# fulcrumgenomics/fgumi

Hardware: AMD Instinct MI355X
Metric: simplex consensus throughput, input raw reads/s (depth-8 x 150bp) (higher is better)
Workload: dtype f64

## Files before the change

### fgumi_amd/csrc/fastpath.hip

```cpp
#if !defined(FGX_WAVEMU)
#include <hipcub/hipcub.hpp>
#endif
#include "bamrec.h"
#include "canon_core.h"
#include "engine.h"
#include <cstdlib>
#include <memory>
#include <string>
#include <type_traits>
#include "fastpath.h"
#include "gate_core.h"
#include "packed_core.h"

#if defined(FGX_WAVEMU)
#define FGX_DYN_LDS(name) uint8_t* const name = wavemu::dyn_lds()
#define FGX_PIN(...) ((void)0)
#define FGX_UNDEF4(a, b, c, d) do { a = 0; b = 0; c = 0; d = 0; } while (0)
#define FGX_MEM_PIN() ((void)0)
#define FGX_CONST_AS
#else
#define FGX_DYN_LDS(name) extern __shared__ __align__(16) uint8_t name[]
#define FGX_PIN(...) asm volatile("" : __VA_ARGS__)
#define FGX_UNDEF4(a, b, c, d) asm volatile("" : "=v"(a), "=v"(b), "=v"(c), "=v"(d))
#define FGX_MEM_PIN() asm volatile("" ::: "memory")
// ... 3219 lines not shown
      FGX_LAUNCH(k_call_full, dim3((mx + 255) / 256, N_LISTS), dim3(256), 0, s, F);
    }
    if (meth_dev) FGX_LAUNCH(k_meth_sizes, dim3((n_slots + 3) / 4), dim3(256), 0, s, P, n_slots, fp.d_mslot.as<MethSlot>());
    if (meth_dup) FGX_LAUNCH(k_duplex_meth_sizes, dim3((n_slots + 3) / 4), dim3(256), 0, s, P, n_slots, fp.d_mslot.as<DuplexMethSlot>());
    return 0;
  }

  int check_direct() {
    FGX_LAUNCH(k_fix_ce, dim3((n_slots + 255) / 256), dim3(256), 0, s, fp.d_slot_desc.as<SlotDesc>(), fp.d_slot_err.as<uint32_t>(), n_slots, fp.d_out.as<uint8_t>(), P.rg_len);
    unsigned long long h_flags = 0, h_def = 0, h_route = 0;
    hip_check(hipMemcpyAsync(&h_flags, misc + MISC_DIR_FLAGS, 8, hipMemcpyDeviceToHost, s), "D2H");
    hip_check(hipMemcpyAsync(&h_def, misc + MISC_N_DEFERRED, 8, hipMemcpyDeviceToHost, s), "D2H");
    hip_check(hipMemcpyAsync(&h_route, misc + MISC_N_ROUTE, 8, hipMemcpyDeviceToHost, s), "D2H");
    hip_check(hipMemcpyAsync(&dir_total, fp.d_dir_base.as<uint64_t>() + fp.dir_chunks_run, 8, hipMemcpyDeviceToHost, s), "D2H");
    sync();
    if ((uint32_t)h_flags != 0) {
      fprintf(stderr, "[fgx] direct records: %u families differ in size from the prediction; this caller goes back to the column scratch (please report)\n", (uint32_t)h_flags);
      fp.direct_off = true;
      return FastPath::RUN_AGAIN_LARGER_POOL;
    }
    if ((uint32_t)(h_flags >> 32) != 0) {
      fp.dir_cap_min = dir_total + dir_total / 16 + 4096;
      if (ps.verbose) fprintf(stderr, "[fgx] direct records: the batch needs %llu bytes of output, %llu were at hand: again\n", (unsigned long long)dir_total, (unsigned long long)dir_cap);
      return FastPath::RUN_AGAIN_LARGER_POOL;
    }
    dir_routed = (uint32_t)h_route;
    dir_pure = dir_routed == 0 && (uint32_t)h_def == 0;
    fp.last_direct = dir_pure ? 1 : 2;
    if (ps.verbose) fprintf(stderr, "[fgx] direct records: %llu bytes in place, %u families left the split pipeline, %u deferred\n", (unsigned long long)dir_total, dir_routed, (uint32_t)h_def);
    return 0;
  }

  void place_records() {
    hip_check(hipEventRecord(fp.ev[1], s), "event");
    out_len = dir_total;
    out_ptr = fp.d_out.as<uint8_t>();
    if (dir_pure) return;
    scan_u64(fp.d_sizes.as<uint64_t>(), fp.d_offsets.as<uint64_t>(), n_slots + 1, "scan");
    uint64_t out_total = 0;
    hip_check(hipMemcpyAsync(&out_total, fp.d_offsets.as<uint64_t>() + n_slots, 8, hipMemcpyDeviceToHost, s), "D2H");
    sync();
    out_len = out_total;
    if (out_len > (1ull << 40)) throw std::runtime_error("device pipeline: the scan of the record sizes gives " + std::to_string(out_len) + " bytes of output (a record size is corrupt)");
    if (direct) { fp.d_out2.reserve(out_len + 16); out_ptr = fp.d_out2.as<uint8_t>(); }
    else { fp.d_out.reserve(out_len + 16); out_ptr = fp.d_out.as<uint8_t>(); }
  }

  template <class EP, class Desc> void emit_params(EP& E, const Desc* ends, uint8_t* out) const {
    memset(&E, 0, sizeof(E));
    E.blob = d_blob; E.rec_off = d_rec_off; E.ends = ends; E.out_off = fp.d_offsets.as<uint64_t>(); E.out = out;
    E.slot_end = n_slots;
    E.col_code = P.col_code; E.col_qual = P.col_qual; E.col_err = P.col_err;
    E.prefix = fp.d_strings.as<char>(); E.prefix_len = P.prefix_len; E.rg = fp.d_strings.as<char>() + P.prefix_len; E.rg_len = P.rg_len;
    E.per_base_tags = P.per_base_tags; E.cell0 = P.cell0; E.cell1 = P.cell1;
  }
  void write_records() {
    hip_check(hipEventRecord(fp.ev[2], s), "event");
    const dim3 per_slot((n_slots + 255) / 256), wave_per_slot((n_slots + 3) / 4), wave_per_family((n_grp + 3) / 4);
    DuplexEmitParams DE;
    CodecEmitParams CE;
    if (codec) {
      emit_params(CE, fp.d_ends.as<CodecDesc>(), fp.d_out.as<uint8_t>());
      CE.col_depth = P.col_depth;
      CE.has_outer = o.codec_has_outer_bases_qual; CE.outer_qual = o.codec_outer_bases_qual; CE.outer_len = o.codec_outer_bases_length;
      CE.has_ss = o.codec_has_single_strand_qual; CE.ss_qual = o.codec_single_strand_qual;
      CE.stats = fp.d_statslots.as<unsigned long long>();
      CE.n_slow = cnt(MISC_N_SLOW);
      FGX_LAUNCH(HIP_KERNEL_NAME(k_count_slow<CodecDesc>), per_slot, dim3(256), 0, s, CE.ends, 0u, n_slots, CE.prefix_len, CE.rg_len, CE.n_slow);
      FGX_LAUNCH(k_emit_codec_fast, wave_per_slot, dim3(256), 0, s, CE);
    } else if (duplex) {
      emit_params(DE, fp.d_ends.as<DuplexDesc>(), fp.d_out.as<uint8_t>());
      DE.col_obs = P.col_obs;
      DE.n_slow = cnt(MISC_N_SLOW);
      DE.meth_flag = P.meth_flag;
      DE.col_obs_all = P.col_obs_all;
      FGX_LAUNCH(HIP_KERNEL_NAME(k_count_slow<DuplexDesc>), per_slot, dim3(256), 0, s, DE.ends, 0u, n_slots, DE.prefix_len, DE.rg_len, DE.n_slow);
      if (meth_dup) FGX_LAUNCH(HIP_KERNEL_NAME(k_emit_duplex_fast<1>), wave_per_slot, dim3(256), 0, s, DE);
      else if (dup_cap) FGX_LAUNCH(HIP_KERNEL_NAME(k_emit_duplex_fast<0, 1>), wave_per_slot, dim3(256), 0, s, DE);
      else FGX_LAUNCH(HIP_KERNEL_NAME(k_emit_duplex_fast<0>), wave_per_slot, dim3(256), 0, s, DE);
    } else if (!direct || !dir_pure) {
      EmitParams E;
      emit_params(E, fp.d_ends.as<EndDesc>(), out_ptr);
      E.col_depth = P.col_depth; E.tag0 = P.tag0; E.tag1 = P.tag1;
      if (!direct) FGX_LAUNCH(k_emit, wave_per_family, dim3(256), 0, s, E);
      else {
        if (dir_routed) {
          E.fam_list = fp.d_route.as<uint32_t>(); E.n_fam = dir_routed;
          FGX_LAUNCH(k_emit, dim3((dir_routed + 3) / 4), dim3(256), 0, s, E);
        }
        FGX_LAUNCH(k_dir_copy, wave_per_family, dim3(256), 0, s, fp.d_split_out.as<SplitOut>(), fp.d_dir_off.as<uint64_t>(), fp.d_offsets.as<uint64_t>(),
                   fp.d_sizes.as<uint64_t>(), fp.d_out.as<uint8_t>(), out_ptr, n_grp);
      }
    }
    if (meth_dev) FGX_LAUNCH(k_meth_tail, wave_per_slot, dim3(256), 0, s, P, n_slots, fp.d_mslot.as<MethSlot>(), fp.d_offsets.as<uint64_t>(), out_ptr);
    if (meth_dup) FGX_LAUNCH(k_duplex_meth_tail, wave_per_slot, dim3(256), 0, s, P, n_slots, fp.d_mslot.as<DuplexMethSlot>(), fp.d_offsets.as<uint64_t>(), out_ptr);
    hip_check(hipEventRecord(fp.ev[3], s), "event");
    hip_check(hipEventRecord(c->ev1, s), "event");
    unsigned long long h_misc[MISC_READ_BACK];
    auto read_counters = [&] {
      FGX_LAUNCH(k_reduce_stats, dim3(1), dim3(64), 0, s, fp.d_statslots.as<unsigned long long>(), misc);
      hip_check(hipMemcpyAsync(h_misc, misc, sizeof(h_misc), hipMemcpyDeviceToHost, s), "D2H");
      sync();
    };
    read_counters();
    if ((duplex || codec) && (uint32_t)h_misc[MISC_N_SLOW] != 0) {
      if (codec) FGX_LAUNCH(k_emit_codec, wave_per_slot, dim3(256), 0, s, CE);
      else if (meth_dup) FGX_LAUNCH(HIP_KERNEL_NAME(k_emit_duplex<1>), wave_per_slot, dim3(256), 0, s, DE);
      else if (dup_cap) FGX_LAUNCH(HIP_KERNEL_NAME(k_emit_duplex<0, 1>), wave_per_slot, dim3(256), 0, s, DE);
      else FGX_LAUNCH(HIP_KERNEL_NAME(k_emit_duplex<0>), wave_per_slot, dim3(256), 0, s, DE);
      read_counters();
    }
    float ms = 0, msf = 0, mse = 0;
    hip_check(hipEventElapsedTime(&ms, c->ev0, c->ev1), "elapsed");
    hip_check(hipEventElapsedTime(&msf, fp.ev[0], fp.ev[1]), "elapsed");
    hip_check(hipEventElapsedTime(&mse, fp.ev[2], fp.ev[3]), "elapsed");
    res->d_out = out_ptr;
    res->out_len = out_len;
    res->count = h_misc[MISC_STATS + 1];
    for (int i = 0; i < FGX_STATS_LEN; i++) res->stats[i] = h_misc[MISC_STATS + i];
    res->n_deferred = (uint32_t)(h_misc[MISC_N_DEFERRED] & 0xFFFFFFFFull);
    fp.last_meth_clipped = (uint32_t)(h_misc[MISC_N_METH_CLIPPED] & 0xFFFFFFFFull);
    res->d_deferred = fp.d_deferred.as<uint32_t>();
    res->d_out_off = fp.d_offsets.as<uint64_t>();
    res->d_slot_size = fp.d_sizes.as<uint64_t>();
    res->n_slots = n_slots;
    res->ms_kernels = ms; res->ms_k_family = msf; res->ms_k_emit = mse;
    fp.last_packed_families = h_misc[MISC_BUILD_FAMILIES]; fp.last_classic_families = h_misc[MISC_BUILD_FAMILIES + 1];
    fp.last_packed_clean = h_misc[MISC_BUILD_FAMILIES + 2]; fp.last_packed_general = h_misc[MISC_BUILD_FAMILIES + 3];
    res->cols_used = h_misc[MISC_COLS_USED];
    res->full_items = n_full;
  }
};

int run_once(FastPath& fp, fgx_caller* c, const uint8_t* d_blob, uint64_t blob_len, const uint64_t* d_rec_off, const uint32_t* d_rec_len, uint32_t n_rec,
             const uint32_t* d_grp_first, uint32_t n_grp, FastResult* res) {
  memset(res, 0, sizeof(*res));
  fp.last_launches = 0; fp.last_host_syncs = 0;
  if (n_grp == 0) return 0;
  static const ProcessSwitches ps{};
  Batch b{fp, c, d_blob, blob_len, d_rec_off, d_rec_len, n_rec, d_grp_first, n_grp, res, ps};
  b.set_up();
  b.parse_first_chunk_early();
  b.bound_columns();
  b.fill_params();
  if (b.use_split) b.split_pipeline();
  if (b.simplex_v2) b.wave2_chain();
  b.family_wave_stages();
  b.deep_families();
  b.workgroup_families();
  if (const int rc = b.call_full()) return rc;
  if (b.direct) if (const int rc = b.check_direct()) return rc;
  b.place_records();
  b.write_records();
  return 0;
}

}

int FastPath::run(fgx_caller* c, const uint8_t* d_blob, uint64_t blob_len, const uint64_t* d_rec_off, const uint32_t* d_rec_len,
                  uint32_t n_rec, const uint32_t* d_grp_first, uint32_t n_grp, FastResult* res) {
  if (!pool_init) {
    if (const char* e = getenv("FGX_POOL_DIV")) { const long v = atol(e); if (v >= 1 && v <= (1 << 20)) pool_div = (uint32_t)v; }
    if (const char* e = getenv("FGX_POOL_SLACK")) { const long v = atol(e); if (v >= 1 && v <= 4096) pool_slack = (uint32_t)v; }
    pool_init = true;
  }
  for (;;) {
    const int rc = run_once(*this, c, d_blob, blob_len, d_rec_off, d_rec_len, n_rec, d_grp_first, n_grp, res);
    if (rc != RUN_AGAIN_LARGER_POOL) {
      if (const char* e = fgx_knob("FGX_S2_DEBUG")) if (atoi(e)) {
        uint32_t h[64];
        if (hipDeviceSynchronize() == hipSuccess && hipMemcpyFromSymbol(h, HIP_SYMBOL(g_s2_dbg), sizeof(h)) == hipSuccess) {
// ... 21 lines not shown
```

### fgumi_amd/csrc/record_writers.inc

```

__device__ __forceinline__ uint8_t int_tag_byte(uint32_t j, char a, char b, uint32_t v) {
  return j == 0 ? (uint8_t)a : j == 1 ? (uint8_t)b : j == 2 ? (uint8_t)(v <= 127 ? 'c' : v <= 255 ? 'C' : 'S') : j == 3 ? (uint8_t)v : (uint8_t)(v >> 8);
}

#ifndef FGX_EMIT_FLAT
#define FGX_EMIT_FLAT 1
#endif
struct EmitCtx {
  uint8_t* q; const uint8_t* first; const uint8_t* code; const uint8_t* cq; const uint16_t* cd; const uint16_t* ce;
  uint32_t Lc, name_len, mi_len, mi_off, flag, rec_size;
};

__device__ __forceinline__ uint32_t gld32u(const uint8_t* p) { uint32_t v; __builtin_memcpy(&v, p, 4); return v; }
__device__ __forceinline__ uint2 gld64u(const uint8_t* p) { uint2 v; __builtin_memcpy(&v, p, 8); return v; }
__device__ __forceinline__ void gst32u(uint8_t* p, uint32_t v) { __builtin_memcpy(p, &v, 4); }
__device__ __forceinline__ void gst16u(uint8_t* p, uint32_t v) { const uint16_t w = (uint16_t)v; __builtin_memcpy(p, &w, 2); }

struct FieldWriterNested {
  uint8_t* q; uint32_t lane;
  static __device__ __forceinline__ uint8_t head3(uint32_t i, char t0, char t1) { return i == 0 ? (uint8_t)t0 : i == 1 ? (uint8_t)t1 : (uint8_t)'Z'; }
  static __device__ __forceinline__ uint8_t head8(uint32_t i, char t0, char t1, uint32_t L) {
    return i == 0 ? (uint8_t)t0 : i == 1 ? (uint8_t)t1 : i == 2 ? (uint8_t)'B' : i == 3 ? (uint8_t)'s' : (uint8_t)(L >> (8 * ((i - 4) & 3)));
  }
  template <class F> __device__ __forceinline__ void small(uint32_t n, F f) { if (lane < n) q[lane] = f(lane); q += n; }
// ... 205 lines not shown
  q += Lc;
#if FGX_EMIT_FLAT
  {
    const uint32_t b = ztag('R' | ('G' << 8) | ('Z' << 16), P.rg_len, R.rgb);
    if (lane < 3 + P.rg_len + 1) q[lane] = (uint8_t)b;
  }
  q += 3 + P.rg_len + 1;
  {
    const uint32_t n3 = n_cd + n_cm + 7, nh = P.per_base_tags ? 8u : 0u;
    auto int_word = [](uint32_t a, uint32_t b, uint32_t v) -> unsigned long long {
      const uint32_t ty = v <= 127 ? (uint32_t)'c' : v <= 255 ? (uint32_t)'C' : (uint32_t)'S';
      return (unsigned long long)(a | (b << 8) | (ty << 16)) | ((unsigned long long)v << 24);
    };
    const unsigned long long w_cd = int_word('c', 'D', maxd), w_cm = int_word('c', 'M', mind);
    const unsigned long long w_ce = (unsigned long long)('c' | ('E' << 8) | ('f' << 16)) | ((unsigned long long)__float_as_uint(ce_rate) << 24);
    const unsigned long long w_hd = (unsigned long long)('c' | ('d' << 8) | ('B' << 16) | ('s' << 24)) | ((unsigned long long)Lc << 32);
    unsigned long long w = w_hd;
    uint32_t k = lane - n3;
    if (lane < n3) { w = w_ce; k = lane - n_cd - n_cm; }
    if (lane < n_cd + n_cm) { w = w_cm; k = lane - n_cd; }
    if (lane < n_cd) { w = w_cd; k = lane; }
    const uint32_t b = (uint32_t)(w >> (8u * (k & 7u)));
    if (lane < n3 + nh) q[lane] = (uint8_t)b;
    q += n3;
  }
#else
  if (lane < 3 + P.rg_len + 1) q[lane] = lane == 0 ? 'R' : lane == 1 ? 'G' : lane == 2 ? 'Z' : j3 < P.rg_len ? R.rgb : (uint8_t)0;
  q += 3 + P.rg_len + 1;
  {
    const uint32_t n3 = n_cd + n_cm + 7, nh = P.per_base_tags ? 8u : 0u;
    if (lane < n3 + nh) {
      const uint32_t i = lane - n3;
      q[lane] = lane < n3 ? cdcmce_byte(lane, n_cd, n_cm, maxd, mind, ce_rate)
                          : (uint8_t)(i == 0 ? 'c' : i == 1 ? 'd' : i == 2 ? 'B' : i == 3 ? 's' : (Lc >> (8 * (i - 4))));
    }
    q += n3;
  }
#endif
  if (P.per_base_tags) {
    q += 8;
#pragma unroll
    for (int t = 0; t < 2; t++) if (4 * (lane + 64 * t) < 2 * Lc) gst32u(q + R.ao[t], R.dw[t]);
    q += 2 * Lc;
    if (lane < 2) gst32u(q + 4 * lane, lane == 0 ? ('c' | ('e' << 8) | ('B' << 16) | ('s' << 24)) : Lc);
    q += 8;
#pragma unroll
    for (int t = 0; t < 2; t++) if (4 * (lane + 64 * t) < 2 * Lc) gst32u(q + R.ao[t], R.ew[t]);
    q += 2 * Lc;
  }
#if FGX_EMIT_FLAT
  {
    const uint32_t b = ztag((uint32_t)(uint8_t)P.tag0 | ((uint32_t)(uint8_t)P.tag1 << 8) | ('Z' << 16), mi_len, R.mib);
    if (lane < 3 + mi_len + 1) q[lane] = (uint8_t)b;
  }
  q += 3 + mi_len + 1;
  if (has_cb) {
    const uint32_t b = ztag((uint32_t)(uint8_t)P.cell0 | ((uint32_t)(uint8_t)P.cell1 << 8) | ('Z' << 16), cb_len, R.cbb);
    if (lane < 3 + cb_len + 1) q[lane] = (uint8_t)b;
    q += 3 + cb_len + 1;
  }
  if (has_rx) {
    const uint32_t b = ztag('R' | ('X' << 8) | ('Z' << 16), rx_len, R.rxb);
    if (lane < 3 + rx_len + 1) q[lane] = (uint8_t)b;
  }
  (void)j3;
#else
  if (lane < 3 + mi_len + 1) q[lane] = lane == 0 ? (uint8_t)P.tag0 : lane == 1 ? (uint8_t)P.tag1 : lane == 2 ? 'Z' : j3 < mi_len ? R.mib : (uint8_t)0;
  q += 3 + mi_len + 1;
  if (has_cb) { if (lane < 3 + cb_len + 1) q[lane] = lane == 0 ? (uint8_t)P.cell0 : lane == 1 ? (uint8_t)P.cell1 : lane == 2 ? 'Z' : j3 < cb_len ? R.cbb : (uint8_t)0; q += 3 + cb_len + 1; }
  if (has_rx) { if (lane < 3 + rx_len + 1) q[lane] = lane == 0 ? 'R' : lane == 1 ? 'X' : lane == 2 ? 'Z' : j3 < rx_len ? R.rxb : (uint8_t)0; }
#endif
}

#ifndef FGX_EMIT_PAIR
#define FGX_EMIT_PAIR 1
#endif
typedef unsigned short em_u16x2 __attribute__((ext_vector_type(2)));
__device__ __forceinline__ uint32_t em_pkmax(uint32_t a, uint32_t b) { em_u16x2 x, y; __builtin_memcpy(&x, &a, 4); __builtin_memcpy(&y, &b, 4); x = __builtin_elementwise_max(x, y); uint32_t r; __builtin_memcpy(&r, &x, 4); return r; }
__device__ __forceinline__ uint32_t em_pkmin(uint32_t a, uint32_t b) { em_u16x2 x, y; __builtin_memcpy(&x, &a, 4); __builtin_memcpy(&y, &b, 4); x = __builtin_elementwise_min(x, y); uint32_t r; __builtin_memcpy(&r, &x, 4); return r; }
__device__ __forceinline__ uint32_t em_sum2(uint32_t pair, uint32_t acc) { em_u16x2 x; const em_u16x2 one = {1, 1}; __builtin_memcpy(&x, &pair, 4); return __builtin_amdgcn_udot2(x, one, acc, false); }
#define FGX_HALF_REDUCE(v, idn, OP) do { \
    v = OP(v, wave_dpp<0xB1, 0xF>(idn, v)); v = OP(v, wave_dpp<0x4E, 0xF>(idn, v)); v = OP(v, wave_dpp<0x141, 0xF>(idn, v)); v = OP(v, wave_dpp<0x140, 0xF>(idn, v)); \
    v = OP(v, wave_dpp<0x142, 0xA>(idn, v)); } while (0)
__device__ __forceinline__ bool emit_pair(const EmitParams& P, const EndDesc* D , uint64_t oo1, uint64_t oo2, uint32_t lane) {
  typedef uint32_t u32x4 __attribute__((ext_vector_type(4)));
  const EndDesc& D1 = D[1];
  const EndDesc& D2 = D[2];
  const uint32_t Lc1 = uni(D1.cons_len), Lc2 = uni(D2.cons_len);
  const uint32_t mi_len = uni(D1.mi_len), mi_off = uni(D1.mi_off);
  const uint64_t first_off = uniform_u64(D1.first_off);
  const uint64_t col1 = uniform_u64(D1.col_off), col2 = uniform_u64(D2.col_off);
  const bool hcb1 = uni(D1.has_cb) != 0, hcb2 = uni(D2.has_cb) != 0, hrx1 = uni(D1.has_rx) != 0, hrx2 = uni(D2.has_rx) != 0;
  const uint32_t cbl1 = hcb1 ? uni(D1.cb_len) : 0u, cbl2 = hcb2 ? uni(D2.cb_len) : 0u, rxl1 = hrx1 ? uni(D1.rx_len) : 0u, rxl2 = hrx2 ? uni(D2.rx_len) : 0u;
  const uint32_t name_len = P.prefix_len + 1u + mi_len, rg_len = P.rg_len;
  const bool ok = Lc1 >= 8u && Lc1 <= 256u && Lc2 >= 8u && Lc2 <= 256u && name_len + 1u <= 32u && rg_len + 4u <= 32u && mi_len + 4u <= 32u &&
                  cbl1 + 4u <= 32u && cbl2 + 4u <= 32u && rxl1 + 4u <= 32u && rxl2 + 4u <= 32u && rxl1 <= (uint32_t)FAST_RX_CAP && rxl2 <= (uint32_t)FAST_RX_CAP &&
                  uniform_u64(D2.first_off) == first_off && uni(D2.mi_len) == mi_len && uni(D2.mi_off) == mi_off &&
                  col2 >= col1 && col2 - col1 < (1ull << 30) && oo2 > oo1 && oo2 - oo1 < (1ull << 30);
  if (!ok) return false;
  const uint32_t l = lane & 31u;
  const bool hb = lane >= 32u;
  const uint32_t Lc = hb ? Lc2 : Lc1;
  const uint32_t dcol = hb ? (uint32_t)(col2 - col1) : 0u, dq = hb ? (uint32_t)(oo2 - oo1) : 0u;
  const uint32_t ty1 = uni(D1.type), ty2 = uni(D2.type), rs1 = uni(D1.rec_size), rs2 = uni(D2.rec_size);
  const uint32_t d_type = hb ? ty2 : ty1, rec_size = hb ? rs2 : rs1;
  const bool hcb = hb ? hcb2 : hcb1, hrx = hb ? hrx2 : hrx1;
  const uint32_t cb_len = hb ? cbl2 : cbl1, rx_len = hb ? rxl2 : rxl1;
  const uint32_t n0 = 8u * l;
  const bool pay = n0 < Lc;
  const uint32_t c0 = min(n0, Lc - 8u);
  const uint32_t cs = min(n0, ((Lc + 1u) & ~1u) - 8u);
  const uint8_t* const code = P.col_code + col1;
  const uint8_t* const cq = P.col_qual + col1;
  const uint8_t* const cdb = (const uint8_t*)(P.col_depth + col1);
  const uint8_t* const ceb = (const uint8_t*)(P.col_err + col1);
  const uint2 cw = gld64u(code + (dcol + cs));
  const uint2 qw = gld64u(cq + (dcol + c0));
  u32x4 dv, ev;
  __builtin_memcpy(&dv, cdb + 2u * (dcol + c0), 16);
  __builtin_memcpy(&ev, ceb + 2u * (dcol + c0), 16);
  const uint8_t* const first = P.blob + first_off;
  const uint32_t j3 = l >= 3u ? l - 3u : 0u;
  const uint32_t ni = l > P.prefix_len ? l - P.prefix_len - 1u : 0u;
  const uint8_t pfx = (uint8_t)P.prefix[l < P.prefix_len ? l : 0u];
  const uint8_t nmb = first[mi_off + (ni < mi_len ? ni : mi_len)];
  const uint8_t rgb = (uint8_t)P.rg[j3 < rg_len ? j3 : 0u];
  const uint8_t mib = first[mi_off + (j3 < mi_len ? j3 : mi_len)];
  uint8_t cbb = 0;
  if (hcb1 || hcb2) {
    const uint64_t k1 = hcb1 ? uniform_u64(D1.kept_off) + uni(D1.cb_off) : first_off, k2 = hcb2 ? uniform_u64(D2.kept_off) + uni(D2.cb_off) : first_off;
    const uint8_t* const fk = P.blob + (hb ? k2 : k1);
    cbb = fk[j3 < cb_len ? j3 : 0u];
  }
  const uint8_t rxb = (uint8_t)D[hb ? 2 : 1].rx[j3 < (uint32_t)FAST_RX_CAP ? j3 : 0u];
  uint32_t maxd, mind, sumd = 0, sume = 0;
  {
    const uint32_t skip16 = 16u * (n0 - c0);
    const uint32_t d4[4] = {dv.x, dv.y, dv.z, dv.w}, e4[4] = {ev.x, ev.y, ev.z, ev.w};
#pragma unroll
    for (int k = 0; k < 4; k++) {
      const int32_t sb = (int32_t)skip16 - 32 * k;
      const uint32_t m = sb <= 0 ? 0xFFFFFFFFu : sb == 16 ? 0xFFFF0000u : 0u;
      sumd = em_sum2(d4[k] & m, sumd); sume = em_sum2(e4[k] & m, sume);
    }
    const uint32_t mx = em_pkmax(em_pkmax(d4[0], d4[1]), em_pkmax(d4[2], d4[3])), mn = em_pkmin(em_pkmin(d4[0], d4[1]), em_pkmin(d4[2], d4[3]));
    maxd = max(mx & 0xFFFFu, mx >> 16); mind = min(mn & 0xFFFFu, mn >> 16);
    if (!pay) { maxd = 0u; mind = 0xFFFFFFFFu; sumd = 0u; sume = 0u; }
  }
  FGX_HALF_REDUCE(maxd, 0u, wr_max); FGX_HALF_REDUCE(mind, 0xFFFFFFFFu, wr_min); FGX_HALF_REDUCE(sumd, 0u, wr_add); FGX_HALF_REDUCE(sume, 0u, wr_add);
  {
    const uint32_t mx0 = rlane(maxd, 31), mx1 = rlane(maxd, 63), mn0 = rlane(mind, 31), mn1 = rlane(mind, 63);
    const uint32_t sd0 = rlane(sumd, 31), sd1 = rlane(sumd, 63), se0 = rlane(sume, 31), se1 = rlane(sume, 63);
    maxd = hb ? mx1 : mx0; mind = hb ? mn1 : mn0; sumd = hb ? sd1 : sd0; sume = hb ? se1 : se0;
  }
  const float ce_rate = sumd > 0u ? (float)sume / (float)sumd : 0.0f;
  const uint32_t n_cd = 3u + int_tag_width(maxd), n_cm = 3u + int_tag_width(mind);
  const uint32_t seq_bytes = (Lc + 1u) >> 1;
  const uint32_t o_seq = dq + 36u + name_len + 1u, o_qual = o_seq + seq_bytes, o_rg = o_qual + Lc, o_t3 = o_rg + 3u + rg_len + 1u;
  const uint32_t n3 = n_cd + n_cm + 7u, nh = P.per_base_tags ? 8u : 0u;
  const uint32_t o_cd = o_t3 + n3 + 8u, o_ceh = o_cd + 2u * Lc, o_ce = o_ceh + 8u;
  const uint32_t o_mi = P.per_base_tags ? o_ce + 2u * Lc : o_t3 + n3;
  const uint32_t o_cb = o_mi + 3u + mi_len + 1u, o_rx = o_cb + (hcb ? 3u + cb_len + 1u : 0u);
  uint8_t* const q = P.out + (oo1 - P.out_base);
  const uint32_t l3 = l < 3u ? l : 3u, sh3 = 8u * l3;
  auto ztag = [&](uint32_t c3, uint32_t len, uint32_t body) -> uint32_t { const uint32_t u = (l - 3u < len) ? body : 0u; return (c3 >> sh3) | u; };
  {
    uint32_t flag = bam::F_UNMAPPED;
    if (d_type == 1u) flag |= bam::F_PAIRED | bam::F_FIRST | bam::F_MATE_UNMAPPED;
    else if (d_type == 2u) flag |= bam::F_PAIRED | bam::F_LAST | bam::F_MATE_UNMAPPED;
    uint32_t v = 0xFFFFFFFFu;
    if (l == 0u) v = rec_size;
    if (l == 3u) v = (name_len + 1u) | (4680u << 16);
    if (l == 4u) v = flag << 16;
    if (l == 5u) v = Lc;
    if (l == 8u) v = 0u;
    if (l < 9u) gst32u(q + (dq + 4u * l), v);
  }
  if (l < name_len + 1u) {
    const uint8_t colon_or_mi = l == P.prefix_len ? (uint8_t)':' : nmb;
    q[dq + 36u + l] = l < P.prefix_len ? pfx : colon_or_mi;
  }
  if (pay) {
    uint32_t lo4 = cw.x, hi4 = cw.y;
    if (cs + 7u >= Lc) hi4 &= 0x00FFFFFFu;
    const uint32_t t = (lo4 << 4) | (lo4 >> 8), u = (hi4 << 4) | (hi4 >> 8);
    gst32u(q + (o_seq + (cs >> 1)), __builtin_amdgcn_perm(u, t, 0x06040200u));
    __builtin_memcpy(q + (o_qual + c0), &qw, 8);
  }
  {
    const uint32_t b = ztag('R' | ('G' << 8) | ('Z' << 16), rg_len, rgb);
    if (l < 3u + rg_len + 1u) q[o_rg + l] = (uint8_t)b;
  }
  {
    auto int_word = [](uint32_t a, uint32_t b, uint32_t v) -> unsigned long long {
      const uint32_t ty = v <= 127u ? (uint32_t)'c' : v <= 255u ? (uint32_t)'C' : (uint32_t)'S';
      return (unsigned long long)(a | (b << 8) | (ty << 16)) | ((unsigned long long)v << 24);
    };
    const unsigned long long w_cd = int_word('c', 'D', maxd), w_cm = int_word('c', 'M', mind);
    const unsigned long long w_ce = (unsigned long long)('c' | ('E' << 8) | ('f' << 16)) | ((unsigned long long)__float_as_uint(ce_rate) << 24);
    const unsigned long long w_hd = (unsigned long long)('c' | ('d' << 8) | ('B' << 16) | ('s' << 24)) | ((unsigned long long)Lc << 32);
    unsigned long long w = w_hd;
    uint32_t k = l - n3;
    if (l < n3) { w = w_ce; k = l - n_cd - n_cm; }
    if (l < n_cd + n_cm) { w = w_cm; k = l - n_cd; }
    if (l < n_cd) { w = w_cd; k = l; }
    const uint32_t b = (uint32_t)(w >> (8u * (k & 7u)));
    if (l < n3 + nh) q[o_t3 + l] = (uint8_t)b;
  }
  if (P.per_base_tags) {
    if (pay) __builtin_memcpy(q + (o_cd + 2u * c0), &dv, 16);
    if (l < 2u) gst32u(q + (o_ceh + 4u * l), l == 0u ? ('c' | ('e' << 8) | ('B' << 16) | ('s' << 24)) : Lc);
    if (pay) __builtin_memcpy(q + (o_ce + 2u * c0), &ev, 16);
  }
  {
    const uint32_t b = ztag((uint32_t)(uint8_t)P.tag0 | ((uint32_t)(uint8_t)P.tag1 << 8) | ('Z' << 16), mi_len, mib);
    if (l < 3u + mi_len + 1u) q[o_mi + l] = (uint8_t)b;
  }
  if (hcb1 || hcb2) {
    const uint32_t b = ztag((uint32_t)(uint8_t)P.cell0 | ((uint32_t)(uint8_t)P.cell1 << 8) | ('Z' << 16), cb_len, cbb);
    if (hcb && l < 3u + cb_len + 1u) q[o_cb + l] = (uint8_t)b;
  }
  if (hrx1 || hrx2) {
    const uint32_t b = ztag('R' | ('X' << 8) | ('Z' << 16), rx_len, rxb);
    if (hrx && l < 3u + rx_len + 1u) q[o_rx + l] = (uint8_t)b;
  }
  return true;
}
#ifndef FGX_EMIT_OCC
#define FGX_EMIT_OCC 7
#endif
__global__ __launch_bounds__(256, FGX_EMIT_OCC) void k_emit(EmitParams P) {
  __shared__ __align__(16) EndDesc sD[4][3];
  static_assert(sizeof(EndDesc) == 96, "EndDesc is copied as six 16-byte pieces");
  uint32_t fam = (uint32_t)__builtin_amdgcn_readfirstlane((int)((blockIdx.x * blockDim.x + threadIdx.x) >> 6));
  const uint32_t lane = threadIdx.x & 63, wv = (threadIdx.x >> 6) & 3;
  if (P.fam_list) {
    if (fam >= P.n_fam) return;
    fam = (uint32_t)__builtin_amdgcn_readfirstlane((int)P.fam_list[fam]);
  }
  const uint32_t s0 = P.slot0 + 3 * fam;
  if (s0 >= P.slot_end) return;
#if defined(FGX_WAVEMU)
#define K_EMIT_PIN(x) ((void)(x))
#else
#define K_EMIT_PIN(x) asm volatile("" :: "s"(x))
#endif
  K_EMIT_PIN(P.blob); K_EMIT_PIN(P.out); K_EMIT_PIN(P.out_base); K_EMIT_PIN(P.col_code); K_EMIT_PIN(P.col_qual); K_EMIT_PIN(P.col_depth);
  K_EMIT_PIN(P.col_err); K_EMIT_PIN(P.prefix); K_EMIT_PIN(P.prefix_len); K_EMIT_PIN(P.rg); K_EMIT_PIN(P.rg_len);
#undef K_EMIT_PIN
  const uint32_t ns = P.slot_end - s0 < 3 ? P.slot_end - s0 : 3;
  typedef uint32_t u32x4 __attribute__((ext_vector_type(4)));
  const u32x4 piece = ((const u32x4*)&P.ends[s0])[lane < 6 * ns ? lane : 0u];
  const uint64_t oo = P.out_off[s0 + (lane < ns ? lane : 0u)];
  if (lane < 6 * ns) ((u32x4*)&sD[wv][0])[lane] = piece;
  wave_sync();
  const bool v0 = uni(sD[wv][0].valid) != 0, v1 = ns > 1 && uni(sD[wv][1].valid) != 0, v2 = ns > 2 && uni(sD[wv][2].valid) != 0;
  auto off_of = [&](int k) -> uint64_t {
    return ((uint64_t)(uint32_t)__builtin_amdgcn_readlane((int)(uint32_t)(oo >> 32), k) << 32) | (uint32_t)__builtin_amdgcn_readlane((int)(uint32_t)oo, k);
  };
  if (v0) { EmitLoads R0; emit_load(P, sD[wv][0], off_of(0), lane, R0); emit_store(P, sD[wv][0], lane, R0); }
#if FGX_EMIT_PAIR
  if (!v0 && v1 && v2 && emit_pair(P, &sD[wv][0], off_of(1), off_of(2), lane)) return;
#endif
  EmitLoads R1, R2;
  if (v1) emit_load(P, sD[wv][1], off_of(1), lane, R1);
  if (v2) emit_load(P, sD[wv][2], off_of(2), lane, R2);
  if (v1) emit_store(P, sD[wv][1], lane, R1);
  if (v2) emit_store(P, sD[wv][2], lane, R2);
}

constexpr uint32_t DUP_SLOTS = 2;

__device__ __forceinline__ bool small_tags(uint32_t name_len, uint32_t mi_len, uint32_t cb_len, uint32_t rg_len, uint32_t rx_len) {
  return name_len + 1 <= 64 && mi_len + 4 <= 64 && cb_len + 4 <= 64 && rg_len + 4 <= 64 && rx_len + 4 <= 64;
}
__device__ __forceinline__ bool fast_ok(const DuplexDesc& D, uint32_t prefix_len, uint32_t rg_len) {
  return D.len <= 128 * DUP_SLOTS && small_tags(prefix_len + 1 + D.mi_len, D.mi_len, D.has_cb ? D.cb_len : 0, rg_len, D.has_rx ? D.rx_len : 0);
}
__device__ __forceinline__ bool fast_ok(const CodecDesc& D, uint32_t prefix_len, uint32_t rg_len) {
  return small_tags(prefix_len + 1 + D.mi_len, D.mi_len, D.has_cb ? D.cb_len : 0, rg_len, D.has_rx ? D.rx_len : 0);
}

__device__ __forceinline__ uint32_t obs_sum(uint32_t o) { return (o & 0xFF) + ((o >> 8) & 0xFF) + ((o >> 16) & 0xFF) + (o >> 24); }
__device__ __forceinline__ uint32_t obs_of_code(uint32_t o, uint32_t code) {
  return code == 1 ? (o & 0xFF) : code == 2 ? ((o >> 8) & 0xFF) : code == 4 ? ((o >> 16) & 0xFF) : code == 8 ? (o >> 24) : 0u;
}
__device__ __forceinline__ uint32_t cap_q(int32_t v) { return v < 2 ? 2u : v > 93 ? 93u : (uint32_t)v; }
template <int METH>
__device__ __forceinline__ void duplex_combine(uint32_t ca, uint32_t qa, uint32_t cb, uint32_t qb, bool ref_c, uint32_t& rb, uint32_t& rq, bool& artifact) {
  artifact = false;
  if constexpr (METH != 0) {
    const uint32_t both = ca | cb;
    artifact = ref_c && ca != cb && (both == 10u || both == 5u);
    if (artifact) { rb = both == 10u ? 2u : 4u; rq = cap_q((int32_t)qa + (int32_t)qb); return; }
  }
  if (ca == cb) { rb = ca; rq = cap_q((int32_t)qa + (int32_t)qb); }
  else if (qa > qb) { rb = ca; rq = cap_q((int32_t)qa - (int32_t)qb); }
  else if (qb > qa) { rb = cb; rq = cap_q((int32_t)qb - (int32_t)qa); }
  else { rb = ca; rq = FGX_MIN_PHRED; }
}
struct DCall { uint32_t rb, oc, oq; bool artifact; };
template <int METH>
__device__ __forceinline__ DCall duplex_call(uint32_t ca, uint32_t qa, uint32_t cb, uint32_t qb, bool ref_c) {
  DCall r;
  uint32_t rq;
  duplex_combine<METH>(ca, qa, cb, qb, ref_c, r.rb, rq, r.artifact);
  const bool nocall = ca == 15 || cb == 15 || rq == FGX_MIN_PHRED;
  r.oc = nocall ? 15u : r.rb; r.oq = nocall ? (uint32_t)FGX_MIN_PHRED : rq;
  return r;
}
__device__ __forceinline__ uint32_t duplex_errors(const DCall& d, uint32_t total, uint32_t xa, uint32_t xb) {
  return (d.rb == 15 || d.artifact) ? 0u : total - (obs_of_code(xa, d.rb) + obs_of_code(xb, d.rb));
}
struct DCol { uint32_t ca, qa, ea, da, cb, qb, eb, db, oc, oq, oe; };
template <int METH>
__device__ __forceinline__ DCol duplex_column(uint32_t ca, uint32_t qa, uint32_t ea, uint32_t oa, bool has_ba, uint32_t cb, uint32_t qb, uint32_t eb, uint32_t ob,
                                              uint32_t xa, uint32_t xb, bool ref_c) {
  DCol c;
  c.ca = ca; c.qa = qa; c.ea = ea; c.da = obs_sum(oa);
  c.cb = 15; c.qb = 0; c.eb = 0; c.db = 0; c.oc = ca; c.oq = qa; c.oe = ea;
  if (has_ba) {
    c.cb = cb; c.qb = qb; c.eb = eb; c.db = obs_sum(ob);
    const DCall d = duplex_call<METH>(ca, qa, cb, qb, ref_c);
    c.oc = d.oc; c.oq = d.oq;
    c.oe = duplex_errors(d, obs_sum(xa) + obs_sum(xb), xa, xb);
  }
  return c;
}

template <int METH, int CAP = 0>
__global__ __launch_bounds__(256) void k_emit_duplex(DuplexEmitParams P) {
  const uint32_t slot = (uint32_t)__builtin_amdgcn_readfirstlane((int)(P.slot0 + ((blockIdx.x * blockDim.x + threadIdx.x) >> 6)));
  const uint32_t lane = threadIdx.x & 63;
  if (slot >= P.slot_end) return;
  const DuplexDesc& D = P.ends[slot];
  if (!D.valid || fast_ok(D, P.prefix_len, P.rg_len)) return;
  const uint32_t L = D.len;
  const bool has_ba = D.has_ba != 0;
  const uint64_t a_off = D.a_off, b_off = D.b_off;
  const uint8_t* mi = P.blob + P.rec_off[D.first_rec] + D.mi_off;
  const uint32_t mi_len = D.mi_len, name_len = P.prefix_len + 1 + mi_len;
  const uint32_t flag = bam::F_UNMAPPED | bam::F_PAIRED | bam::F_MATE_UNMAPPED | (D.type == 1 ? bam::F_FIRST : bam::F_LAST);
  auto col = [&](uint32_t i) {
    const uint64_t ia = a_off + i, ib = b_off + i;
    const uint32_t oa = P.col_obs[ia];
    uint32_t cb = 15, qb = 0, eb = 0, ob = 0, xa = oa, xb = 0;
    bool ref_c = false;
    if (has_ba) {
      cb = P.col_code[ib]; qb = P.col_qual[ib]; eb = P.col_err[ib]; ob = P.col_obs[ib]; xb = ob;
      if constexpr (METH != 0) ref_c = (P.meth_flag[ia] | P.meth_flag[ib]) != 0;
      if constexpr (CAP != 0) { if (D.capped) { xa = P.col_obs_all[ia]; xb = P.col_obs_all[ib]; } }
// ... 419 lines not shown
```

Before: 2.928 billion.

## Process multiple families per wavefront in k_emit and split pair-emit into load/store phases

The emit kernel now has each wavefront handle FGX_EMIT_FAMS (default 2) families instead of one. The paired-end emit is split into a load phase and a store phase, so global loads for all families in the wave are issued before any stores, raising memory-level parallelism. Descriptor staging in LDS is widened to match, and the launch grid shrinks accordingly. The cost is more registers per wave, so the launch-bounds occupancy target drops from 7 to 5, and the fallback path for unpaired families becomes a per-family loop.

```diff
diff --git a/fgumi_amd/csrc/fastpath.hip b/fgumi_amd/csrc/fastpath.hip
--- a/fgumi_amd/csrc/fastpath.hip
+++ b/fgumi_amd/csrc/fastpath.hip
@@ -3325,11 +3325,12 @@
       EmitParams E;
       emit_params(E, fp.d_ends.as<EndDesc>(), out_ptr);
       E.col_depth = P.col_depth; E.tag0 = P.tag0; E.tag1 = P.tag1;
-      if (!direct) FGX_LAUNCH(k_emit, wave_per_family, dim3(256), 0, s, E);
+      auto wave_per_group = [](uint32_t n_fam) { return dim3(((n_fam + FGX_EMIT_FAMS - 1) / FGX_EMIT_FAMS + 3) / 4); };
+      if (!direct) FGX_LAUNCH(k_emit, wave_per_group(n_grp), dim3(256), 0, s, E);
       else {
         if (dir_routed) {
           E.fam_list = fp.d_route.as<uint32_t>(); E.n_fam = dir_routed;
-          FGX_LAUNCH(k_emit, dim3((dir_routed + 3) / 4), dim3(256), 0, s, E);
+          FGX_LAUNCH(k_emit, wave_per_group(dir_routed), dim3(256), 0, s, E);
         }
         FGX_LAUNCH(k_dir_copy, wave_per_family, dim3(256), 0, s, fp.d_split_out.as<SplitOut>(), fp.d_dir_off.as<uint64_t>(), fp.d_offsets.as<uint64_t>(),
                    fp.d_sizes.as<uint64_t>(), fp.d_out.as<uint8_t>(), out_ptr, n_grp);
diff --git a/fgumi_amd/csrc/record_writers.inc b/fgumi_amd/csrc/record_writers.inc
--- a/fgumi_amd/csrc/record_writers.inc
+++ b/fgumi_amd/csrc/record_writers.inc
@@ -311,8 +311,16 @@
 #define FGX_HALF_REDUCE(v, idn, OP) do { \
     v = OP(v, wave_dpp<0xB1, 0xF>(idn, v)); v = OP(v, wave_dpp<0x4E, 0xF>(idn, v)); v = OP(v, wave_dpp<0x141, 0xF>(idn, v)); v = OP(v, wave_dpp<0x140, 0xF>(idn, v)); \
     v = OP(v, wave_dpp<0x142, 0xA>(idn, v)); } while (0)
-__device__ __forceinline__ bool emit_pair(const EmitParams& P, const EndDesc* D , uint64_t oo1, uint64_t oo2, uint32_t lane) {
-  typedef uint32_t u32x4 __attribute__((ext_vector_type(4)));
+typedef uint32_t em_u32x4 __attribute__((ext_vector_type(4)));
+struct PairLoads {
+  uint64_t oo1;
+  uint32_t Lc1, Lc2, mi_len, dq2, ty1, ty2, rs1, rs2, cbl1, cbl2, rxl1, rxl2;
+  bool hcb1, hcb2, hrx1, hrx2;
+  uint2 cw, qw; em_u32x4 dv, ev;
+  uint8_t pfx, nmb, rgb, mib, cbb, rxb;
+};
+__device__ __forceinline__ bool emit_pair_load(const EmitParams& P, const EndDesc* D , uint64_t oo1, uint64_t oo2, uint32_t lane, PairLoads& R) {
+  typedef em_u32x4 u32x4;
   const EndDesc& D1 = D[1];
   const EndDesc& D2 = D[2];
   const uint32_t Lc1 = uni(D1.cons_len), Lc2 = uni(D2.cons_len);
@@ -330,11 +338,9 @@
   const uint32_t l = lane & 31u;
   const bool hb = lane >= 32u;
   const uint32_t Lc = hb ? Lc2 : Lc1;
-  const uint32_t dcol = hb ? (uint32_t)(col2 - col1) : 0u, dq = hb ? (uint32_t)(oo2 - oo1) : 0u;
+  const uint32_t dcol = hb ? (uint32_t)(col2 - col1) : 0u;
   const uint32_t ty1 = uni(D1.type), ty2 = uni(D2.type), rs1 = uni(D1.rec_size), rs2 = uni(D2.rec_size);
-  const uint32_t d_type = hb ? ty2 : ty1, rec_size = hb ? rs2 : rs1;
-  const bool hcb = hb ? hcb2 : hcb1, hrx = hb ? hrx2 : hrx1;
-  const uint32_t cb_len = hb ? cbl2 : cbl1, rx_len = hb ? rxl2 : rxl1;
+  const uint32_t cb_len = hb ? cbl2 : cbl1;
   const uint32_t n0 = 8u * l;
   const bool pay = n0 < Lc;
   const uint32_t c0 = min(n0, Lc - 8u);
@@ -362,6 +368,33 @@
     cbb = fk[j3 < cb_len ? j3 : 0u];
   }
   const uint8_t rxb = (uint8_t)D[hb ? 2 : 1].rx[j3 < (uint32_t)FAST_RX_CAP ? j3 : 0u];
+  R.oo1 = oo1; R.dq2 = (uint32_t)(oo2 - oo1);
+  R.Lc1 = Lc1; R.Lc2 = Lc2; R.mi_len = mi_len; R.ty1 = ty1; R.ty2 = ty2; R.rs1 = rs1; R.rs2 = rs2;
+  R.cbl1 = cbl1; R.cbl2 = cbl2; R.rxl1 = rxl1; R.rxl2 = rxl2; R.hcb1 = hcb1; R.hcb2 = hcb2; R.hrx1 = hrx1; R.hrx2 = hrx2;
+  R.cw = cw; R.qw = qw; R.dv = dv; R.ev = ev;
+  R.pfx = pfx; R.nmb = nmb; R.rgb = rgb; R.mib = mib; R.cbb = cbb; R.rxb = rxb;
+  return true;
+}
+__device__ __forceinline__ void emit_pair_store(const EmitParams& P, uint32_t lane, const PairLoads& R) {
+  typedef em_u32x4 u32x4;
+  const uint32_t Lc1 = R.Lc1, Lc2 = R.Lc2, mi_len = R.mi_len;
+  const bool hcb1 = R.hcb1, hcb2 = R.hcb2, hrx1 = R.hrx1, hrx2 = R.hrx2;
+  const uint32_t name_len = P.prefix_len + 1u + mi_len, rg_len = P.rg_len;
+  const uint32_t l = lane & 31u;
+  const bool hb = lane >= 32u;
+  const uint32_t Lc = hb ? Lc2 : Lc1;
+  const uint32_t dq = hb ? R.dq2 : 0u;
+  const uint32_t d_type = hb ? R.ty2 : R.ty1, rec_size = hb ? R.rs2 : R.rs1;
+  const bool hcb = hb ? hcb2 : hcb1, hrx = hb ? hrx2 : hrx1;
+  const uint32_t cb_len = hb ? R.cbl2 : R.cbl1, rx_len = hb ? R.rxl2 : R.rxl1;
+  const uint32_t n0 = 8u * l;
+  const bool pay = n0 < Lc;
+  const uint32_t c0 = min(n0, Lc - 8u);
+  const uint32_t cs = min(n0, ((Lc + 1u) & ~1u) - 8u);
+  const uint2 cw = R.cw, qw = R.qw;
+  const u32x4 dv = R.dv, ev = R.ev;
+  const uint8_t pfx = R.pfx, nmb = R.nmb, rgb = R.rgb, mib = R.mib, cbb = R.cbb, rxb = R.rxb;
+  const uint64_t oo1 = R.oo1;
   uint32_t maxd, mind, sumd = 0, sume = 0;
   {
     const uint32_t skip16 = 16u * (n0 - c0);
@@ -453,22 +486,22 @@
     const uint32_t b = ztag('R' | ('X' << 8) | ('Z' << 16), rx_len, rxb);
     if (hrx && l < 3u + rx_len + 1u) q[o_rx + l] = (uint8_t)b;
   }
-  return true;
-}
+}
+#ifndef FGX_EMIT_FAMS
+#define FGX_EMIT_FAMS 2
+#endif
 #ifndef FGX_EMIT_OCC
-#define FGX_EMIT_OCC 7
+#define FGX_EMIT_OCC (FGX_EMIT_FAMS == 1 ? 7 : FGX_EMIT_FAMS == 2 ? 5 : 3)
 #endif
+static_assert(FGX_EMIT_FAMS >= 1 && FGX_EMIT_FAMS <= 4, "k_emit: the output offsets of a wavefront's families lie in the lanes of one register (3 * 18 + 2 < 64)");
 __global__ __launch_bounds__(256, FGX_EMIT_OCC) void k_emit(EmitParams P) {
-  __shared__ __align__(16) EndDesc sD[4][3];
+  constexpr uint32_t F = FGX_EMIT_FAMS, PIECES = 18 * F, ROUNDS = (PIECES + 63) / 64;
+  __shared__ __align__(16) EndDesc sD[4][F][3];
   static_assert(sizeof(EndDesc) == 96, "EndDesc is copied as six 16-byte pieces");
-  uint32_t fam = (uint32_t)__builtin_amdgcn_readfirstlane((int)((blockIdx.x * blockDim.x + threadIdx.x) >> 6));
+  const uint32_t grp = (uint32_t)__builtin_amdgcn_readfirstlane((int)((blockIdx.x * blockDim.x + threadIdx.x) >> 6));
   const uint32_t lane = threadIdx.x & 63, wv = (threadIdx.x >> 6) & 3;
-  if (P.fam_list) {
-    if (fam >= P.n_fam) return;
-    fam = (uint32_t)__builtin_amdgcn_readfirstlane((int)P.fam_list[fam]);
-  }
-  const uint32_t s0 = P.slot0 + 3 * fam;
-  if (s0 >= P.slot_end) return;
+  const uint32_t n_list = P.fam_list ? P.n_fam : (P.slot_end - P.slot0 + 2) / 3;
+  if (F * grp >= n_list || P.slot0 >= P.slot_end) return;
 #if defined(FGX_WAVEMU)
 #define K_EMIT_PIN(x) ((void)(x))
 #else
@@ -477,25 +510,51 @@
   K_EMIT_PIN(P.blob); K_EMIT_PIN(P.out); K_EMIT_PIN(P.out_base); K_EMIT_PIN(P.col_code); K_EMIT_PIN(P.col_qual); K_EMIT_PIN(P.col_depth);
   K_EMIT_PIN(P.col_err); K_EMIT_PIN(P.prefix); K_EMIT_PIN(P.prefix_len); K_EMIT_PIN(P.rg); K_EMIT_PIN(P.rg_len);
 #undef K_EMIT_PIN
-  const uint32_t ns = P.slot_end - s0 < 3 ? P.slot_end - s0 : 3;
   typedef uint32_t u32x4 __attribute__((ext_vector_type(4)));
-  const u32x4 piece = ((const u32x4*)&P.ends[s0])[lane < 6 * ns ? lane : 0u];
-  const uint64_t oo = P.out_off[s0 + (lane < ns ? lane : 0u)];
-  if (lane < 6 * ns) ((u32x4*)&sD[wv][0])[lane] = piece;
+  uint64_t oo = 0;
+#pragma unroll
+  for (uint32_t t = 0; t < ROUNDS; t++) {
+    const uint32_t i = lane + 64 * t, j = i / 18, pc = i - 18 * j, e = F * grp + j;
+    const bool listed = i < PIECES && e < n_list;
+    const uint32_t fam = P.fam_list ? P.fam_list[listed ? e : F * grp] : e;
+    const uint32_t slot = P.slot0 + 3 * fam + pc / 6;
+    const bool in = listed && slot < P.slot_end;
+    const u32x4 piece = ((const u32x4*)&P.ends[in ? P.slot0 + 3 * fam : P.slot0])[in ? pc : 0u];
+    if (t == 0) oo = P.out_off[in && pc < 3 && P.slot0 + 3 * fam + pc < P.slot_end ? P.slot0 + 3 * fam + pc : P.slot0];
+    const u32x4 zero = {0u, 0u, 0u, 0u};
+    if (i < PIECES) ((u32x4*)&sD[wv][0][0])[i] = in ? piece : zero;
+  }
   wave_sync();
-  const bool v0 = uni(sD[wv][0].valid) != 0, v1 = ns > 1 && uni(sD[wv][1].valid) != 0, v2 = ns > 2 && uni(sD[wv][2].valid) != 0;
-  auto off_of = [&](int k) -> uint64_t {
-    return ((uint64_t)(uint32_t)__builtin_amdgcn_readlane((int)(uint32_t)(oo >> 32), k) << 32) | (uint32_t)__builtin_amdgcn_readlane((int)(uint32_t)oo, k);
+  auto off_of = [&](uint32_t j, uint32_t k) -> uint64_t {
+    return ((uint64_t)(uint32_t)__builtin_amdgcn_readlane((int)(uint32_t)(oo >> 32), 18 * j + k) << 32) | (uint32_t)__builtin_amdgcn_readlane((int)(uint32_t)oo, 18 * j + k);
   };
-  if (v0) { EmitLoads R0; emit_load(P, sD[wv][0], off_of(0), lane, R0); emit_store(P, sD[wv][0], lane, R0); }
+  uint32_t rest = 0;
+#pragma unroll
+  for (uint32_t j = 0; j < F; j++) rest |= 1u << j;
 #if FGX_EMIT_PAIR
-  if (!v0 && v1 && v2 && emit_pair(P, &sD[wv][0], off_of(1), off_of(2), lane)) return;
+  PairLoads L[F];
+#pragma unroll
+  for (uint32_t j = 0; j < F; j++) {
+    const EndDesc* D = &sD[wv][j][0];
+    if (__builtin_expect(uni(D[0].valid) == 0 && uni(D[1].valid) != 0 && uni(D[2].valid) != 0 && emit_pair_load(P, D, off_of(j, 1), off_of(j, 2), lane, L[j]), 1)) rest &= ~(1u << j);
+  }
+#pragma unroll
+  for (uint32_t j = 0; j < F; j++)
+    if (!(rest & (1u << j))) emit_pair_store(P, lane, L[j]);
 #endif
-  EmitLoads R1, R2;
-  if (v1) emit_load(P, sD[wv][1], off_of(1), lane, R1);
-  if (v2) emit_load(P, sD[wv][2], off_of(2), lane, R2);
-  if (v1) emit_store(P, sD[wv][1], lane, R1);
-  if (v2) emit_store(P, sD[wv][2], lane, R2);
+  if (__builtin_expect(rest == 0, 1)) return;
+#pragma unroll
+  for (uint32_t j = 0; j < F; j++) {
+    if (!(rest & (1u << j))) continue;
+    const EndDesc* D = &sD[wv][j][0];
+    const bool v0 = uni(D[0].valid) != 0, v1 = uni(D[1].valid) != 0, v2 = uni(D[2].valid) != 0;
+    if (v0) { EmitLoads R0; emit_load(P, D[0], off_of(j, 0), lane, R0); emit_store(P, D[0], lane, R0); }
+    EmitLoads R1, R2;
+    if (v1) emit_load(P, D[1], off_of(j, 1), lane, R1);
+    if (v2) emit_load(P, D[2], off_of(j, 2), lane, R2);
+    if (v1) emit_store(P, D[1], lane, R1);
+    if (v2) emit_store(P, D[2], lane, R2);
+  }
 }
 
 constexpr uint32_t DUP_SLOTS = 2;
```

Measured after the change: 2.977 billion, median of 6. +1.7%, better.
